# ChristophReich1996/Semantic_Pyramid_for_Image_Generation

Hardware: AMD Instinct MI355X
Metric: images/sec full G+D train step, 256x256, bs/GPU=20 (higher is better)
Workload: dtype bf16

## Files before the change

semantic_pyramid_for_image_generation_amd/csrc/conv_igemm.hip:

```cpp
#include "conv_common.h"

namespace {

template <typename T, int WCO, int WPX, int FCO, int FPX>
__global__ __launch_bounds__(256) void conv_igemm_kernel(sp_conv_params p) {
    constexpr int CO_T = WCO * FCO * 16, PX_T = WPX * FPX * 16;
    constexpr int E = 16 / (int)sizeof(T);
    constexpr int KC = 8 * E;
    constexpr int W_CH = CO_T * 8, X_CH = PX_T * 8;
    constexpr int W_PER = (W_CH + 255) / 256, X_PER = (X_CH + 255) / 256;
    constexpr int STAGE = (CO_T + PX_T) * 128;
    extern __shared__ __attribute__((aligned(16))) char smem[];

    const int tid = threadIdx.x, lane = tid & 63, wave = tid >> 6;
    const int wco = wave / WPX, wpx = wave % WPX;
    const int H = p.h, W = p.w_, CIN = p.cin_p;
    const long M = (long)p.n * H * W;
    const long px0 = (long)blockIdx.x * PX_T;
    const int co0 = blockIdx.y * CO_T;
    const int taps = p.ksize * p.ksize;
    const int kchunks = (CIN + KC - 1) / KC;
    const int nk = taps * kchunks;
    const T* __restrict__ xg = reinterpret_cast<const T*>(p.x);
    const T* __restrict__ wg = reinterpret_cast<const T*>(p.w);
// ... 675 lines not shown
        const unsigned add = c0 + ls < CIN ? (unsigned)(c0 * (int)sizeof(T)) : OOB_C;
        char* dst = halo_l + (gc & 1) * HALO_BUF + wave * 6 * 1024;
#pragma unroll
        for (int i = 0; i < 6; ++i) {
            if (wave * 6 + i < HALO_INSTR)
                __builtin_amdgcn_raw_ptr_buffer_load_lds(x_rsrc, (__attribute__((address_space(3))) void*)(dst + i * 1024), 16,
                                                         (int)(h_off[i] + add), 0, 0, 0);
        }
    };
    auto issue_w = [&](int gc, int ds, int buf) {
        const int c0 = (gc % kchunks) * KC;
        const unsigned base = (unsigned)(((TPS == 9 ? 0 : ds) * CIN + c0) * (int)sizeof(T));
        char* dst = wbuf_l + buf * W_BYTES + wave * W_PER * 1024;
#pragma unroll
        for (int i = 0; i < W_PER; ++i) {
            if (wave * W_PER + i < W_INSTR) {
                const unsigned add = c0 + w_ls(i) < CIN ? base : OOB_C;
                __builtin_amdgcn_raw_ptr_buffer_load_lds(w_rsrc, (__attribute__((address_space(3))) void*)(dst + i * 1024), 16,
                                                         (int)(w_off[i] + add), 0, 0, 0);
            }
        }
    };

    const int frow = lane & 15, fslot = lane >> 4;
    const unsigned a_addr = lds_base + 2 * HALO_BUF + (wco * 64 + (frow >> 2) * 16 + (frow & 3)) * 64 +
                            ((fslot ^ (((frow >> 1) & 1) | (((frow >> 2) & 1) << 1))) << 4);
    unsigned b_addr[3];
#pragma unroll
    for (int ds = 0; ds < 3; ++ds)
        b_addr[ds] = lds_base + ((RW * wpx) * HP + frow + ds) * 64 + ((fslot ^ (((frow + ds) >> 1) & 3)) << 4);

    const bool bias_in_acc = p.bias != nullptr && !up && p.img_scale == nullptr;
    f32x4_t acc[4][NFR];
    auto init_acc = [&](int it) {
        f32x4_t b4[4];
#pragma unroll
        for (int i = 0; i < 4; ++i) b4[i] = f32x4_t{0.f, 0.f, 0.f, 0.f};
        if (bias_in_acc && it < my_items) {
            int n, ty0, tx0, co0;
            item_coords(it, n, ty0, tx0, co0);
            const int cb = co0 + wco * 64 + (lane >> 4) * 16;
#pragma unroll
            for (int i = 0; i < 4; ++i) {
                const int co = cb + i * 4;
                if (co + 3 < p.cout) {
                    const float4 t = *reinterpret_cast<const float4*>(p.bias + co);
                    b4[i] = f32x4_t{t.x, t.y, t.z, t.w};
                } else {
#pragma unroll
                    for (int r = 0; r < 4; ++r) b4[i][r] = co + r < p.cout ? p.bias[co + r] : 0.f;
                }
            }
        }
#pragma unroll
        for (int i = 0; i < 4; ++i)
#pragma unroll
            for (int j = 0; j < NFR; ++j) acc[i][j] = b4[i];
    };
    init_acc(0);

    constexpr int IH = (WCO == 2 && RW == 4) ? 2 : 1, IW = 4 / IH;
    auto stage = [&](auto ds_c, unsigned ab, unsigned bb, auto&& mid) {
        constexpr int DS = decltype(ds_c)::value;
        constexpr int TAP_STRIDE = CO_T * 64;
        constexpr int A0 = (TPS == 9 ? DS : 0) * TAP_STRIDE, ADR = (TPS == 9 ? 3 : 1) * TAP_STRIDE;
        const unsigned bo = HP == 36 ? (bb ^ 32u) : bb;
        static_for<IH>([&](auto ihc) {
            constexpr int i0 = decltype(ihc)::value * IW;
            uint4 a[3][IW], bf[NB][2];
            static_for<IW>([&](auto i) { lds_rd128<A0 + (i0 + decltype(i)::value) * 256>(a[0][decltype(i)::value], ab); });
            lds_rd128<0>(bf[0][0], bb); lds_rd128<1024>(bf[0][1], bb);
            static_for<NB>([&](auto hc) {
                constexpr int h = decltype(hc)::value;
                if constexpr (h + 1 < NB) {
                    if constexpr (h + 1 < 3)
                        static_for<IW>([&](auto i) { lds_rd128<A0 + (h + 1) * ADR + (i0 + decltype(i)::value) * 256>(a[h + 1][decltype(i)::value], ab); });
                    lds_rd128<(h + 1) * (HP * 64)>(bf[h + 1][0], ((h + 1) & 1) ? bo : bb);
                    lds_rd128<(h + 1) * (HP * 64) + 1024>(bf[h + 1][1], ((h + 1) & 1) ? bo : bb);
                    wait_lgkm<(h + 1 < 3) ? IW + 2 : 2>();
                } else {
                    wait_lgkm<0>();
                }
                static_for<3>([&](auto drc) {
                    constexpr int dr = decltype(drc)::value;
                    constexpr int rr = h - dr;
                    if constexpr (rr >= 0 && rr < RW) {
#pragma unroll
                        for (int i = 0; i < IW; ++i)
#pragma unroll
                            for (int hh = 0; hh < 2; ++hh) Mma<T>::run(a[dr][i], bf[h][hh], acc[i0 + i][rr * 2 + hh]);
                    }
                });
                if constexpr (h == 1 && decltype(ihc)::value == 0) mid();
            });
        });
    };

    if (nchunks <= 0) return;
    const bool late = stagger != 0 && wave >= 4;
    set_halo_desc(0);
    set_w_desc(0);
    issue_halo(0);
    issue_w(0, 0, 0);
    int g = 0;
    int kc = 0, item = 0;
    const bool vec_ok = ((p.ldy & 3) == 0) && ((p.cout & 3) == 0);
    for (int gc = 0; gc < nchunks; ++gc) {
        const bool more_chunks = gc + 1 < nchunks;
        const bool item_ends = kc + 1 == kchunks;
        const unsigned hb = (unsigned)((gc & 1) * HALO_BUF);
        static_for<SPC>([&](auto sc) {
            constexpr int st = decltype(sc)::value;
            wait_vmcnt<0>();
            __builtin_amdgcn_s_barrier();
            auto request = [&]() {
                if (st + 1 < SPC) {
                    issue_w(gc, st + 1, (g + 1) & 1);
                } else if (more_chunks) {
                    if (item_ends) set_w_desc(item + 1);
                    issue_w(gc + 1, 0, (g + 1) & 1);
                }
                if (st == 0 && more_chunks) {
                    if (item_ends) set_halo_desc(item + 1);
                    issue_halo(gc + 1);
                }
            };
            if (!late) request();
            const unsigned ab = a_addr + (unsigned)((g & 1) * W_BYTES);
            auto deferred = [&]() { if (late) request(); };
            auto nothing = []() {};
            if constexpr (SPC == 3) {
                stage(std::integral_constant<int, st>{}, ab, b_addr[st] + hb, deferred);
            } else {
                stage(std::integral_constant<int, 0>{}, ab, b_addr[0] + hb, deferred);
                stage(std::integral_constant<int, 1>{}, ab, b_addr[1] + hb, nothing);
                stage(std::integral_constant<int, 2>{}, ab, b_addr[2] + hb, nothing);
            }
            ++g;
        });
        if (item_ends) {
            int n, ty0, tx0, co0;
            item_coords(item, n, ty0, tx0, co0);
            const long pix0 = ((long)n * H + ty0 + RW * wpx) * W + tx0 + (lane & 15);
            const int co_b = co0 + wco * 64 + (lane >> 4) * 16;
            const bool wide = vec_ok && (p.ldy & 7) == 0 && co_b + 16 <= p.cout;
            if (up) {
#pragma unroll
                for (int i = 0; i < 4; ++i)
#pragma unroll
                    for (int j = 0; j < NFR; ++j) acc[i][j] *= 0.25f;
            }
            static_for<NFR>([&](auto jc) {
                constexpr int j = decltype(jc)::value;
                const long pix = pix0 + (long)(j >> 1) * W + (j & 1) * 16;
                if (p.pool2) {
                    if constexpr ((j & 3) == 0) {
                        const long prow = ((long)n * (H >> 1) + ((ty0 + RW * wpx + (j >> 1)) >> 1)) * (W >> 1);
                        if constexpr (IDX) {
                            float a0[16], a1[16], b0[16], b1[16];
#pragma unroll
                            for (int i = 0; i < 4; ++i)
#pragma unroll
                                for (int r = 0; r < 4; ++r) {
                                    a0[i * 4 + r] = acc[i][j][r]; a1[i * 4 + r] = acc[i][j + 2][r];
                                    b0[i * 4 + r] = acc[i][j + 1][r]; b1[i * 4 + r] = acc[i][j + 3][r];
                                }
                            conv_epilogue_pool2_idx<T>(p, a0, a1, b0, b1, lane, prow, tx0 >> 1, co_b, !bias_in_acc);
                        } else {
                            float a[16], b[16];
#pragma unroll
                            for (int i = 0; i < 4; ++i)
#pragma unroll
                                for (int r = 0; r < 4; ++r) {
                                    a[i * 4 + r] = pool2_combine(acc[i][j][r], acc[i][j + 2][r], p.pool2 == 2);
                                    b[i * 4 + r] = pool2_combine(acc[i][j + 1][r], acc[i][j + 3][r], p.pool2 == 2);
                                }
                            conv_epilogue_pool2<T>(p, a, b, lane, prow, tx0 >> 1, co_b, !bias_in_acc);
                        }
                    }
                } else if (wide) {
                    float v[16];
#pragma unroll
                    for (int i = 0; i < 4; ++i)
#pragma unroll
                        for (int r = 0; r < 4; ++r) v[i * 4 + r] = acc[i][j][r];
                    conv_epilogue16<T>(p, v, pix, co_b, !bias_in_acc);
                } else {
#pragma unroll
                    for (int i = 0; i < 4; ++i) {
                        const int co = co_b + i * 4;
                        if (co < p.cout) {
                            float v[4] = {acc[i][j][0], acc[i][j][1], acc[i][j][2], acc[i][j][3]};
                            conv_epilogue4<T>(p, v, pix, co, vec_ok, !bias_in_acc);
                        }
                    }
                }
            });
            kc = 0;
            ++item;
            init_acc(item);
        } else {
            ++kc;
        }
    }
}

template <typename T, int WCO, int TH = 16, bool IDX = false>
int launch_tall(const sp_conv_params& p, hipStream_t s) {
    constexpr int HP = WCO == 1 ? 36 : 40;
    constexpr int LDS = 2 * ((((TH + 2) * HP * 64 + 1023) / 1024) * 1024) + 2 * (WCO == 1 ? 9 : 3) * 64 * WCO * 64;
    constexpr auto kern = conv3x3_tall_kernel<T, WCO, TH, IDX>;
    if (const int rc = sp_lds_limit<kern>(LDS)) return rc;
    const int cotiles = (p.cout + 64 * WCO - 1) / (64 * WCO);
    const int total = p.n * (p.h / TH) * (p.w_ / TL_TW) * cotiles;
    int grid = total < NUM_CU ? total : NUM_CU;
    if (grid >= 8) grid -= grid % 8;
    sp_note_route(conv_route_name(WCO == 1 ? CK_TALL_1_16 : TH == 16 ? CK_TALL_2_16 : CK_TALL_2_8, 0, sizeof(T) == 4));
    hipLaunchKernelGGL(kern, dim3((unsigned)grid), dim3(512), LDS, s, p, cotiles, total, sp_tune(SP_TUNE_CONV_STAGGER, (WCO == 2 && TH == 16) ? 1 : 0));
    SP_LAUNCH_CHECK();
    return SP_OK;
}

inline int igemm_nk(int cin_p, int ksize, int dtype) {
    const int e = dtype == SP_F32 ? 4 : 8;
    return ksize * ksize * ((cin_p + 8 * e - 1) / (8 * e));
}
inline int igemm_small_tile(long M, int cout, int cin_p, int ksize, int dtype) {
    const int forced = sp_tune(SP_TUNE_IGEMM_TILE, -1);
    if (forced >= 0) return forced;
    const long tiles64 = ((M + 63) / 64) * ((cout + 63) / 64);
    return (tiles64 > 256 && tiles64 <= 512 && igemm_nk(cin_p, ksize, dtype) >= 48 && cout % 128 == 0) ? 2 : 0;
}
struct IgemmTile { int co_t, px_t; };
constexpr int tile_key(int co_t, int px_t) { return co_t * 1024 + px_t; }
inline IgemmTile igemm_tile(bool dma, long M, int cout, int cin_p, int ksize, int dtype) {
    if (cout <= 64) return {cout <= 16 ? 16 : cout <= 32 ? 32 : 64, 256};
    if (M > 8192) return {128, 128};
    switch (dma ? igemm_small_tile(M, cout, cin_p, ksize, dtype) : 0) {
        case 1: return {128, 128};
        case 2: return {128, 64};
        case 3: return {64, 128};
        default: return {64, 64};
    }
}

inline int split_k_plan(int tiles, int nk) {
    const int target = sp_tune(SP_TUNE_SPLITK_TARGET, 384);
    int min_steps = sp_tune(SP_TUNE_SPLITK_MINSTEPS, 6);
    if (min_steps < 1) min_steps = 1;
    if (tiles > 256 || nk < 16) return 1;
    int ksplit = (target + tiles - 1) / tiles;
    if (ksplit > nk / min_steps) ksplit = nk / min_steps;
    if (ksplit > 16) ksplit = 16;
    return ksplit < 1 ? 1 : ksplit;
}
inline int igemm_ksplit_wanted(IgemmTile t, long M, int cout, int cin_p, int ksize, int dtype) {
    return split_k_plan((int)((M + t.px_t - 1) / t.px_t) * ((cout + t.co_t - 1) / t.co_t), igemm_nk(cin_p, ksize, dtype));
}
inline int igemm_ksplit(const sp_conv_params& p, IgemmTile t) {
    const long M = (long)p.n * p.h * p.w_;
    int ksplit = p.workspace == nullptr ? 1 : igemm_ksplit_wanted(t, M, p.cout, p.cin_p, p.ksize, p.dtype);
    while (ksplit > 1 && p.workspace_bytes < (int64_t)ksplit * M * p.cout * 4) --ksplit;
    if (ksplit > 1) {
        const int nk = igemm_nk(p.cin_p, p.ksize, p.dtype), per = (nk + ksplit - 1) / ksplit;
        ksplit = (nk + per - 1) / per;
    }
    return ksplit;
}

template <typename T, int WCO, int WPX, int FCO, int FPX>
int launch_dma(const sp_conv_params& p, int ksplit, hipStream_t s) {
    constexpr int CO_T = WCO * FCO * 16, PX_T = WPX * FPX * 16;
    constexpr int LDS = 3 * (CO_T + PX_T) * 128;
    constexpr auto kern = conv_igemm_dma_kernel<T, WCO, WPX, FCO, FPX>;
    if (const int rc = sp_lds_limit<kern>(LDS)) return rc;
    const long M = (long)p.n * p.h * p.w_;
    dim3 grid((unsigned)((M + PX_T - 1) / PX_T), (unsigned)((p.cout + CO_T - 1) / CO_T), (unsigned)ksplit);
    sp_note_route(conv_route_name(CK_IGEMM_DMA, ksplit > 1 ? CV_SPLITK : 0, false));
    hipLaunchKernelGGL(kern, grid, dim3(256), LDS, s, p, ksplit);
    SP_LAUNCH_CHECK();
    if (ksplit > 1) {
        long blocks = (M * ((p.cout + 3) / 4) + 255) / 256;
        if (blocks > 1024) blocks = 1024;
        hipLaunchKernelGGL(conv_finalize_kernel<T>, dim3((unsigned)blocks), dim3(256), 0, s, p, ksplit);
        SP_LAUNCH_CHECK();
    }
    return SP_OK;
}

template <typename T, int WCO, int WPX, int FCO, int FPX>
int launch_cfg(const sp_conv_params& p, hipStream_t s) {
    constexpr int CO_T = WCO * FCO * 16, PX_T = WPX * FPX * 16;
    constexpr int LDS = 2 * (CO_T + PX_T) * 128;
    constexpr auto kern = conv_igemm_kernel<T, WCO, WPX, FCO, FPX>;
    if (const int rc = sp_lds_limit<kern>(LDS)) return rc;
    const long M = (long)p.n * p.h * p.w_;
    dim3 grid((unsigned)((M + PX_T - 1) / PX_T), (unsigned)((p.cout + CO_T - 1) / CO_T));
    sp_note_route(conv_route_name(CK_IGEMM, 0, false));
    hipLaunchKernelGGL(kern, grid, dim3(256), LDS, s, p);
    SP_LAUNCH_CHECK();
    return SP_OK;
}

__global__ __launch_bounds__(256) void conv1x1_direct_kernel(sp_conv_params p, int row_bytes) {
    extern __shared__ __attribute__((aligned(16))) char wsm[];
    const int tid = threadIdx.x, lane = tid & 63, wave = tid >> 6;
    const int CIN = p.cin_p;
    const long M = (long)p.n * p.h * p.w_;
    const int co0 = blockIdx.y * 64;
    const bf16* __restrict__ xg = reinterpret_cast<const bf16*>(p.x);
    const bf16* __restrict__ wg = reinterpret_cast<const bf16*>(p.w);
    const int ksteps = (CIN + 31) / 32;
    const int cpr = ksteps * 4;
    for (int e = tid; e < 64 * cpr; e += 256) {
        const int row = e / cpr, c = e - row * cpr;
        uint4 v = make_uint4(0, 0, 0, 0);
        if (co0 + row < p.cout && c * 8 < CIN) v = *reinterpret_cast<const uint4*>(wg + (long)(co0 + row) * CIN + c * 8);
        *reinterpret_cast<uint4*>(wsm + row * row_bytes + ((c ^ (((row >> 4) & 1) << 2)) << 4)) = v;
    }
    __syncthreads();
    const int i16 = lane & 15, g = lane >> 4;
    const int arow = (i16 >> 2) * 16 + (i16 & 3);
    const int aswz = ((arow >> 4) & 1) << 2;
    const bool vec_ok = ((p.ldy & 3) == 0) && ((p.cout & 3) == 0);
    const int co_b = co0 + g * 16;
    const bool wide = vec_ok && (p.ldy & 7) == 0 && co_b + 16 <= p.cout;
    const long ngroups = (M + 31) / 32;
    for (long grp = (long)blockIdx.x * 4 + wave; grp < ngroups; grp += (long)gridDim.x * 4) {
        const long px0 = grp * 32 + i16, px1 = px0 + 16;
        const bf16* x0 = xg + (px0 < M ? px0 : M - 1) * CIN + g * 8;
        const bf16* x1 = xg + (px1 < M ? px1 : M - 1) * CIN + g * 8;
        f32x4_t acc[4][2];
#pragma unroll
        for (int i = 0; i < 4; ++i) { acc[i][0] = f32x4_t{0.f, 0.f, 0.f, 0.f}; acc[i][1] = f32x4_t{0.f, 0.f, 0.f, 0.f}; }
        for (int m = 0; m < ksteps; ++m) {
            uint4 b0 = make_uint4(0, 0, 0, 0), b1 = make_uint4(0, 0, 0, 0);
            if (m * 32 + g * 8 < CIN) {
                b0 = *reinterpret_cast<const uint4*>(x0 + m * 32);
                b1 = *reinterpret_cast<const uint4*>(x1 + m * 32);
            }
            const int slot = (m * 4 + g) ^ aswz;
#pragma unroll
            for (int i = 0; i < 4; ++i) {
                const uint4 a = *reinterpret_cast<const uint4*>(wsm + (arow + i * 4) * row_bytes + (slot << 4));
                acc[i][0] = __builtin_amdgcn_mfma_f32_16x16x32_bf16(__builtin_bit_cast(bf16x8_t, a), __builtin_bit_cast(bf16x8_t, b0), acc[i][0], 0, 0, 0);
                acc[i][1] = __builtin_amdgcn_mfma_f32_16x16x32_bf16(__builtin_bit_cast(bf16x8_t, a), __builtin_bit_cast(bf16x8_t, b1), acc[i][1], 0, 0, 0);
            }
        }
        static_for<2>([&](auto jc) {
            constexpr int j = decltype(jc)::value;
            const long pix = j == 0 ? px0 : px1;
            if (pix < M) {
                if (wide) {
                    float v[16];
#pragma unroll
                    for (int i = 0; i < 4; ++i)
#pragma unroll
                        for (int r = 0; r < 4; ++r) v[i * 4 + r] = acc[i][j][r];
                    conv_epilogue16<bf16>(p, v, pix, co_b);
                } else {
                    static_for<4>([&](auto ic) {
                        constexpr int i = decltype(ic)::value;
                        const int co = co_b + i * 4;
                        if (co < p.cout) {
                            float v[4] = {acc[i][j][0], acc[i][j][1], acc[i][j][2], acc[i][j][3]};
                            conv_epilogue4<bf16>(p, v, pix, co, vec_ok);
                        }
                    });
                }
            }
        });
    }
}

int launch_1x1_direct(const sp_conv_params& p, hipStream_t s) {
    const int ksteps = (p.cin_p + 31) / 32;
    const int row_bytes = ((ksteps * 64 + 127) / 128) * 128 + 16;
    const int lds = 64 * row_bytes;
    if (const int rc = sp_lds_limit<conv1x1_direct_kernel>(lds)) return rc;
    const long M = (long)p.n * p.h * p.w_;
    const int cotiles = (p.cout + 63) / 64;
    long gx = (M + 127) / 128;
    const long cap = 1024 / cotiles > 0 ? 1024 / cotiles : 1;
    if (gx > cap) gx = cap;
    sp_note_route(conv_route_name(CK_1X1_DIRECT, 0, false));
    hipLaunchKernelGGL(conv1x1_direct_kernel, dim3((unsigned)gx, (unsigned)cotiles), dim3(256), lds, s, p, row_bytes);
    SP_LAUNCH_CHECK();
    return SP_OK;
}


template <int KMAX>
__global__ __launch_bounds__(256) void conv1x1_splitk_kernel(sp_conv_params p) {
    __shared__ float4 red[4 * 4 * 2 * 64];
    const int tid = threadIdx.x, lane = tid & 63, wave = tid >> 6;
    const int CIN = p.cin_p;
    const long M = (long)p.n * p.h * p.w_;
    const int co0 = blockIdx.y * 64;
    const bf16* __restrict__ xg = reinterpret_cast<const bf16*>(p.x);
    const bf16* __restrict__ wg = reinterpret_cast<const bf16*>(p.w);
    const int ksteps = (CIN + 31) / 32;
    const int per = (ksteps + 3) / 4;
    const int m0 = wave * per;
    const int cnt = ksteps - m0 < per ? ksteps - m0 : per;
    const int i16 = lane & 15, g = lane >> 4;
    const int arow = (i16 >> 2) * 16 + (i16 & 3);
    const long px0 = (long)blockIdx.x * 32 + i16, px1 = px0 + 16;
    const bf16* x0 = xg + (px0 < M ? px0 : M - 1) * CIN + g * 8;
    const bf16* x1 = xg + (px1 < M ? px1 : M - 1) * CIN + g * 8;
    const bf16* wr[4];
#pragma unroll
    for (int i = 0; i < 4; ++i) {
        const int row = co0 + arow + i * 4;
        wr[i] = wg + (long)(row < p.cout ? row : p.cout - 1) * CIN + g * 8;
    }
    f32x4_t acc[4][2];
#pragma unroll
    for (int i = 0; i < 4; ++i) { acc[i][0] = f32x4_t{0.f, 0.f, 0.f, 0.f}; acc[i][1] = f32x4_t{0.f, 0.f, 0.f, 0.f}; }
    for (int c0 = 0; c0 < cnt; c0 += KMAX) {
        uint4 a[KMAX][4], b[KMAX][2];
        static_for<KMAX>([&](auto uc) {
            constexpr int u = decltype(uc)::value;
            const int m = m0 + c0 + u;
#pragma unroll
            for (int i = 0; i < 4; ++i) a[u][i] = make_uint4(0, 0, 0, 0);
            b[u][0] = make_uint4(0, 0, 0, 0);
            b[u][1] = make_uint4(0, 0, 0, 0);
            if (c0 + u < cnt && m * 32 + g * 8 < CIN) {
#pragma unroll
                for (int i = 0; i < 4; ++i) a[u][i] = *reinterpret_cast<const uint4*>(wr[i] + m * 32);
                b[u][0] = *reinterpret_cast<const uint4*>(x0 + m * 32);
                b[u][1] = *reinterpret_cast<const uint4*>(x1 + m * 32);
            }
        });
        static_for<KMAX>([&](auto uc) {
            constexpr int u = decltype(uc)::value;
            if (c0 + u < cnt) {
#pragma unroll
                for (int i = 0; i < 4; ++i) {
                    acc[i][0] = __builtin_amdgcn_mfma_f32_16x16x32_bf16(__builtin_bit_cast(bf16x8_t, a[u][i]), __builtin_bit_cast(bf16x8_t, b[u][0]), acc[i][0], 0, 0, 0);
                    acc[i][1] = __builtin_amdgcn_mfma_f32_16x16x32_bf16(__builtin_bit_cast(bf16x8_t, a[u][i]), __builtin_bit_cast(bf16x8_t, b[u][1]), acc[i][1], 0, 0, 0);
                }
            }
        });
    }
#pragma unroll
    for (int i = 0; i < 4; ++i)
#pragma unroll
        for (int j = 0; j < 2; ++j)
            red[((wave * 4 + i) * 2 + j) * 64 + lane] = make_float4(acc[i][j][0], acc[i][j][1], acc[i][j][2], acc[i][j][3]);
    __syncthreads();
    const bool vec_ok = ((p.ldy & 3) == 0) && ((p.cout & 3) == 0);
    const int co = co0 + g * 16 + wave * 4;
    if (co >= p.cout) return;
#pragma unroll
    for (int j = 0; j < 2; ++j) {
        const long pix = j == 0 ? px0 : px1;
        float v[4] = {0.f, 0.f, 0.f, 0.f};
#pragma unroll
        for (int src = 0; src < 4; ++src) {
            const float4 t = red[((src * 4 + wave) * 2 + j) * 64 + lane];
            v[0] += t.x; v[1] += t.y; v[2] += t.z; v[3] += t.w;
        }
        if (pix < M) conv_epilogue4<bf16>(p, v, pix, co, vec_ok);
    }
}

int launch_1x1_splitk(const sp_conv_params& p, hipStream_t s) {
    const int ksteps = (p.cin_p + 31) / 32;
    const long M = (long)p.n * p.h * p.w_;
    dim3 grid((unsigned)((M + 31) / 32), (unsigned)((p.cout + 63) / 64));
    sp_note_route(conv_route_name(CK_1X1_SPLITK, 0, false));
    if (ksteps <= 8) hipLaunchKernelGGL(conv1x1_splitk_kernel<2>, grid, dim3(256), 0, s, p);
    else if (ksteps <= 16) hipLaunchKernelGGL(conv1x1_splitk_kernel<4>, grid, dim3(256), 0, s, p);
    else hipLaunchKernelGGL(conv1x1_splitk_kernel<6>, grid, dim3(256), 0, s, p);
    SP_LAUNCH_CHECK();
    return SP_OK;
}

constexpr int C8_TH = 16, C8_TW = 32, C8_HW = C8_TW + 2, C8_HH = C8_TH + 2;

__global__ __launch_bounds__(256) void conv3x3_cin8_kernel(sp_conv_params p) {
    __shared__ __attribute__((aligned(16))) uint4 halo[C8_HH * C8_HW];
    const int tid = threadIdx.x, lane = tid & 63, wave = tid >> 6;
    const int H = p.h, W = p.w_;
    const int tiles_x = W / C8_TW, tiles_y = H / C8_TH;
    int t = blockIdx.x;
    const int tx0 = (t % tiles_x) * C8_TW; t /= tiles_x;
    const int ty0 = (t % tiles_y) * C8_TH;
    const int n = t / tiles_y;
    const uint4* __restrict__ xg = reinterpret_cast<const uint4*>(p.x);
    const uint4* __restrict__ wg = reinterpret_cast<const uint4*>(p.w);
    uint4 hv[3];
#pragma unroll
    for (int q = 0; q < 3; ++q) {
        const int e = tid + q * 256;
        const int r = e / C8_HW, c = e - r * C8_HW;
        const int y = ty0 - 1 + r, x = tx0 - 1 + c;
        hv[q] = make_uint4(0, 0, 0, 0);
        if (e < C8_HH * C8_HW && (unsigned)y < (unsigned)H && (unsigned)x < (unsigned)W) hv[q] = xg[((long)n * H + y) * W + x];
    }
    const int i16 = lane & 15, g = lane >> 4;
    uint4 a[4][3];
#pragma unroll
    for (int i = 0; i < 4; ++i) {
        const int co = (i16 >> 2) * 16 + i * 4 + (i16 & 3);
#pragma unroll
        for (int m = 0; m < 3; ++m) {
            const int tap = m * 4 + g;
            a[i][m] = make_uint4(0, 0, 0, 0);
            if (tap < 9 && co < p.cout) a[i][m] = wg[co * 9 + tap];
        }
    }
#pragma unroll
    for (int q = 0; q < 3; ++q) {
        const int e = tid + q * 256;
        if (e < C8_HH * C8_HW) halo[e] = hv[q];
    }
    __syncthreads();
    int toff[3];
#pragma unroll
    for (int m = 0; m < 3; ++m) {
        const int tap = m * 4 + g < 9 ? m * 4 + g : 8;
        toff[m] = (tap / 3) * C8_HW + tap % 3;
    }
    const int co_b = g * 16;
    const bool co_ok = co_b + 16 <= p.cout;
    float bias[16];
#pragma unroll
    for (int r = 0; r < 16; ++r) bias[r] = 0.f;
    if (p.bias && co_ok) Wide16<float>::ld(p.bias + co_b, bias);
#pragma unroll 2
    for (int rr = 0; rr < C8_TH / 4; ++rr) {
        const int row = wave * (C8_TH / 4) + rr;
        f32x4_t acc[4][2];
#pragma unroll
        for (int i = 0; i < 4; ++i) { acc[i][0] = f32x4_t{0.f, 0.f, 0.f, 0.f}; acc[i][1] = f32x4_t{0.f, 0.f, 0.f, 0.f}; }
#pragma unroll
        for (int m = 0; m < 3; ++m) {
            const uint4 b0 = halo[row * C8_HW + i16 + toff[m]];
            const uint4 b1 = halo[row * C8_HW + 16 + i16 + toff[m]];
#pragma unroll
            for (int i = 0; i < 4; ++i) {
                acc[i][0] = __builtin_amdgcn_mfma_f32_16x16x32_bf16(__builtin_bit_cast(bf16x8_t, a[i][m]), __builtin_bit_cast(bf16x8_t, b0), acc[i][0], 0, 0, 0);
                acc[i][1] = __builtin_amdgcn_mfma_f32_16x16x32_bf16(__builtin_bit_cast(bf16x8_t, a[i][m]), __builtin_bit_cast(bf16x8_t, b1), acc[i][1], 0, 0, 0);
            }
        }
        if (!co_ok) continue;
        const long pix0 = ((long)n * H + ty0 + row) * W + tx0 + i16;
        const float sc = conv_img_scale(p, pix0);
#pragma unroll
        for (int j = 0; j < 2; ++j) {
            float v[16];
#pragma unroll
            for (int i = 0; i < 4; ++i)
#pragma unroll
                for (int r = 0; r < 4; ++r) v[i * 4 + r] = acc[i][j][r] * sc + bias[i * 4 + r];
            conv_epilogue16<bf16>(p, v, pix0 + j * 16, co_b, false);
        }
    }
}

int launch_cin8(const sp_conv_params& p, hipStream_t s) {
    const long blocks = (long)p.n * (p.h / C8_TH) * (p.w_ / C8_TW);
    sp_note_route(conv_route_name(CK_CIN8, 0, false));
    hipLaunchKernelGGL(conv3x3_cin8_kernel, dim3((unsigned)blocks), dim3(256), 0, s, p);
    SP_LAUNCH_CHECK();
    return SP_OK;
}

constexpr int TN_TH = 8, TN_TW = 32, TN_HW = TN_TW + 2, TN_HH = TN_TH + 2;

template <int KC>
__global__ __launch_bounds__(256) void conv3x3_thinco_kernel(sp_conv_params p) {
    extern __shared__ __attribute__((aligned(16))) char tn_smem[];
    constexpr int CIN = KC * 32, PITCH = CIN * 2 + 16, CPP = KC * 4;
    constexpr int NCH = TN_HH * TN_HW * CPP, PER = (NCH + 255) / 256;
    const int tid = threadIdx.x, lane = tid & 63, wave = tid >> 6;
    const int H = p.h, W = p.w_;
    const int tiles_x = W / TN_TW, tiles_y = H / TN_TH;
    int t = blockIdx.x;
    const int tx0 = (t % tiles_x) * TN_TW; t /= tiles_x;
    const int ty0 = (t % tiles_y) * TN_TH;
    const int n = t / tiles_y;
    const uint4* __restrict__ xg = reinterpret_cast<const uint4*>(p.x);
    const uint4* __restrict__ wg = reinterpret_cast<const uint4*>(p.w);
    uint4 hv[PER];
#pragma unroll
    for (int q = 0; q < PER; ++q) {
        const int e = tid + q * 256;
        const int px = e / CPP, c = e - px * CPP;
        const int r = px / TN_HW, cc = px - r * TN_HW;
        const int y = ty0 - 1 + r, x = tx0 - 1 + cc;
        hv[q] = make_uint4(0, 0, 0, 0);
        if (e < NCH && (unsigned)y < (unsigned)H && (unsigned)x < (unsigned)W) hv[q] = xg[(((long)n * H + y) * W + x) * CPP + c];
    }
    const int i16 = lane & 15, g = lane >> 4;
    uint4 a[9][KC];
#pragma unroll
    for (int tap = 0; tap < 9; ++tap)
#pragma unroll
        for (int kc = 0; kc < KC; ++kc) {
            a[tap][kc] = make_uint4(0, 0, 0, 0);
            if (i16 < p.cout) a[tap][kc] = wg[(i16 * 9 + tap) * CPP + kc * 4 + g];
        }
#pragma unroll
    for (int q = 0; q < PER; ++q) {
        const int e = tid + q * 256;
        const int px = e / CPP, c = e - px * CPP;
        if (e < NCH) *reinterpret_cast<uint4*>(tn_smem + px * PITCH + c * 16) = hv[q];
    }
    __syncthreads();
    const bool vec_ok = ((p.ldy & 3) == 0) && ((p.cout & 3) == 0);
#pragma unroll
    for (int rr = 0; rr < TN_TH / 4; ++rr) {
        const int row = wave * (TN_TH / 4) + rr;
        f32x4_t acc[2] = {f32x4_t{0.f, 0.f, 0.f, 0.f}, f32x4_t{0.f, 0.f, 0.f, 0.f}};
#pragma unroll
        for (int tap = 0; tap < 9; ++tap) {
            const char* base = tn_smem + ((row + tap / 3) * TN_HW + i16 + tap % 3) * PITCH + g * 16;
#pragma unroll
            for (int kc = 0; kc < KC; ++kc) {
                const uint4 b0 = *reinterpret_cast<const uint4*>(base + kc * 64);
                const uint4 b1 = *reinterpret_cast<const uint4*>(base + 16 * PITCH + kc * 64);
                acc[0] = __builtin_amdgcn_mfma_f32_16x16x32_bf16(__builtin_bit_cast(bf16x8_t, a[tap][kc]), __builtin_bit_cast(bf16x8_t, b0), acc[0], 0, 0, 0);
                acc[1] = __builtin_amdgcn_mfma_f32_16x16x32_bf16(__builtin_bit_cast(bf16x8_t, a[tap][kc]), __builtin_bit_cast(bf16x8_t, b1), acc[1], 0, 0, 0);
            }
        }
        if (g != 0) continue;
        const long pix0 = ((long)n * H + ty0 + row) * W + tx0 + i16;
#pragma unroll
        for (int j = 0; j < 2; ++j) {
            float v[4] = {acc[j][0], acc[j][1], acc[j][2], acc[j][3]};
            conv_epilogue4<bf16>(p, v, pix0 + j * 16, 0, vec_ok);
        }
    }
}

template <int KC>
int launch_thinco(const sp_conv_params& p, hipStream_t s) {
    constexpr int LDS = TN_HH * TN_HW * (KC * 64 + 16);
    if (const int rc = sp_lds_limit<conv3x3_thinco_kernel<KC>>(LDS)) return rc;
    const long blocks = (long)p.n * (p.h / TN_TH) * (p.w_ / TN_TW);
    sp_note_route(conv_route_name(CK_THINCO, 0, false));
    hipLaunchKernelGGL(conv3x3_thinco_kernel<KC>, dim3((unsigned)blocks), dim3(256), LDS, s, p);
    SP_LAUNCH_CHECK();
    return SP_OK;
}

inline bool conv_halo_path(long M, int h, int w, int cin_p, int cout, int ksize) {
    const bool thin_big = cout <= 16 && cin_p >= 32 && M >= (1L << 18);
    return ksize == 3 && (cout > 32 || thin_big) && h % HALO_TH == 0 && w % HALO_TW == 0;
}
inline bool conv_w16_path(int w, int cout, int ksize, bool h16) {
    const int ppm = sp_tune(SP_TUNE_CONV_PP, 1);
    return h16 && ksize == 3 && w == 16 && cout > 64 && (ppm == 1 || ppm == 3);
}
inline bool conv_dma_path(long M, int cout, int ksize) {
    const int dma_mode = sp_tune(SP_TUNE_IGEMM_DMA, 1);
    return cout > 16 && (dma_mode == 2 || (dma_mode == 1 && ksize == 3 && M <= 8192));
}

ConvRoute conv_plan(const sp_conv_params& p) {
    const auto route = [](int kernel, int form = 0) { return ConvRoute{kernel, form, 0, 0, 1, nullptr}; };
    const auto unsupported = [](const char* msg) { return ConvRoute{CK_UNSUPPORTED, 0, 0, 0, 1, msg}; };
    int form;
    if (p.dtype == SP_F8) {
        if ((form = sp_conv_pp_form(p, CK_PP_8ROW)) >= 0) return route(CK_PP_8ROW, form);
        return unsupported("sp_conv2d_igemm: SP_F8 covers 3x3 layers with cout > 64, h %% 8 == 0, w %% 32 == 0 only");
    }
    const bool h16 = p.dtype != SP_F32;
    const int esz = h16 ? 2 : 4, idx = p.pool_idx != nullptr ? CV_IDX : 0;
    const int pp_mode = h16 ? sp_tune(SP_TUNE_CONV_PP, 1) : 0, tall_mode = sp_tune(SP_TUNE_CONV_TALL, 1);
    if (p.tail_w != nullptr) {
        if (!p.in_up2 && p.img_scale == nullptr && pp_mode && tall_mode == 1 && (form = sp_conv_pp_form(p, CK_PP_16ROW)) >= 0) return route(CK_PP_16ROW, form);
        return unsupported("sp_conv2d_igemm: the fused 1x1 tail needs 16-bit storage, a 3x3 layer with cout == 64, h %% 16 == 0, w %% 32 == 0, ldy %% 8 == 0, no pooling");
    }
    const long M = (long)p.n * p.h * p.w_;
    if (h16 && p.ksize == 3 && p.cout <= 4 && (p.cin_p == 32 || p.cin_p == 64) && !p.pool2 && !p.in_up2 && p.h % TN_TH == 0 &&
        p.w_ % TN_TW == 0 && sp_tune(SP_TUNE_CONV_THINCO, 1) && tall_mode <= 1)
        return route(CK_THINCO);
    if (h16 && p.ksize == 3 && p.cin_p == 8 && p.cout % 16 == 0 && p.cout <= 64 && (p.ldy & 7) == 0 && !p.pool2 && !p.in_up2 &&
        p.h % C8_TH == 0 && p.w_ % C8_TW == 0 && sp_tune(SP_TUNE_CONV_CIN8, 1) && tall_mode <= 1)
        return route(CK_CIN8);
    if (h16 && p.ksize == 1) {
        const int ks = (p.cin_p + 31) / 32;
        const bool few_blocks = ((M + 31) / 32) * ((p.cout + 63) / 64) <= sp_tune(SP_TUNE_CONV1X1_SPLITK, 320);
        if (few_blocks && (p.cin_p > 1024 || (ks >= 4 && ks <= 24))) return route(CK_1X1_SPLITK);
        if (p.cin_p <= 1024 && sp_tune(SP_TUNE_CONV1X1_DIRECT, 1)) return route(CK_1X1_DIRECT);
    }
    const bool fits30 = conv_operands_below_1g(p, esz);
// ... 158 lines not shown
```

Before: 1366.

## Pipeline 1x1 direct conv with register-prefetched activations and templated K depth

Rewrites the 1x1 direct convolution kernel so the K depth is a template parameter. Activation loads for all K steps are issued into registers up front, and the next pixel group is prefetched while the current epilogue runs; a ring mode streams batches for deep channel counts. Weight loading into LDS is overlapped with the first activation loads, and the grid is sized from the CU count and LDS occupancy instead of a fixed cap. The costs are heavier register pressure, more template instantiations, and reliance on inline asm and sched barriers.

Measured after the change: 1372 (median of 6 runs). About the same (+0.4%).

```diff
diff --git a/semantic_pyramid_for_image_generation_amd/csrc/conv_igemm.hip b/semantic_pyramid_for_image_generation_amd/csrc/conv_igemm.hip
--- a/semantic_pyramid_for_image_generation_amd/csrc/conv_igemm.hip
+++ b/semantic_pyramid_for_image_generation_amd/csrc/conv_igemm.hip
@@ -1001,54 +1001,141 @@
     return SP_OK;
 }
 
-__global__ __launch_bounds__(256) void conv1x1_direct_kernel(sp_conv_params p, int row_bytes) {
+inline long direct1x1_ranges(long M, int cotiles, int lds_bytes) {
+    int per_cu = (160 * 1024) / lds_bytes;
+    per_cu = per_cu > 4 ? 4 : per_cu < 1 ? 1 : per_cu;
+    const long groups = (M + 31) / 32;
+    long ranges = (long)NUM_CU * per_cu / cotiles;
+    if (ranges > 8) ranges &= ~7L;
+    if (ranges > (groups + 3) / 4) ranges = (groups + 3) / 4;
+    return ranges < 1 ? 1 : ranges;
+}
+
+template <int KB, bool RING>
+__global__ __launch_bounds__(256, RING && KB == 8 ? 2 : 4) void conv1x1_direct_kernel(sp_conv_params p, int row_bytes, int nranges, int nbatch) {
     extern __shared__ __attribute__((aligned(16))) char wsm[];
-    const int tid = threadIdx.x, lane = tid & 63, wave = tid >> 6;
+    const int tid = threadIdx.x, lane = tid & 63;
+    const int wave = __builtin_amdgcn_readfirstlane(tid >> 6);
     const int CIN = p.cin_p;
     const long M = (long)p.n * p.h * p.w_;
-    const int co0 = blockIdx.y * 64;
-    const bf16* __restrict__ xg = reinterpret_cast<const bf16*>(p.x);
-    const bf16* __restrict__ wg = reinterpret_cast<const bf16*>(p.w);
-    const int ksteps = (CIN + 31) / 32;
-    const int cpr = ksteps * 4;
-    for (int e = tid; e < 64 * cpr; e += 256) {
-        const int row = e / cpr, c = e - row * cpr;
-        uint4 v = make_uint4(0, 0, 0, 0);
-        if (co0 + row < p.cout && c * 8 < CIN) v = *reinterpret_cast<const uint4*>(wg + (long)(co0 + row) * CIN + c * 8);
-        *reinterpret_cast<uint4*>(wsm + row * row_bytes + ((c ^ (((row >> 4) & 1) << 2)) << 4)) = v;
-    }
+    const int cotiles = (p.cout + 63) >> 6;
+    const int bq = (int)blockIdx.x >> 3;
+    const int range = (bq / cotiles) * 8 + ((int)blockIdx.x & 7);
+    if (range >= nranges) return;
+    const int co0 = (bq % cotiles) * 64;
+    const int ksteps = RING ? nbatch * KB : KB;
+    int i16 = lane & 15, g = lane >> 4;
+    const int ngroups = (int)((M + 31) / 32);
+    const int gstride = nranges * 4;
+    const char* xb;
+    unsigned r0, r1;
+    auto rows_of = [&](int gr) {
+        const long p0 = (long)(gr < ngroups ? gr : ngroups - 1) * 32;
+        const int last = (int)(M - 1 - p0 < 31 ? M - 1 - p0 : 31);
+        xb = reinterpret_cast<const char*>(p.x) + p0 * CIN * 2;
+        r0 = (unsigned)((i16 < last ? i16 : last) * CIN * 2);
+        r1 = (unsigned)((i16 + 16 < last ? i16 + 16 : last) * CIN * 2);
+    };
+    uint4 b[KB][2];
+    auto issue = [&](auto jc, int base, bool may_be_last) {
+        constexpr int j = decltype(jc)::value;
+        unsigned ch = (unsigned)(base + j * 64 + g * 16);
+        if (j == KB - 1 && may_be_last) ch = ch < (unsigned)CIN * 2 ? ch : 0u;
+        b[j][0] = *reinterpret_cast<const uint4*>(xb + (r0 + ch));
+        b[j][1] = *reinterpret_cast<const uint4*>(xb + (r1 + ch));
+    };
+    constexpr int NF = RING ? 4 : (KB + 1) / 2;
+    const int kpieces = (ksteps + 1) / 2;
+    const int frow = tid >> 3, fswz = ((frow >> 4) & 1) << 2;
+    const char* wb = reinterpret_cast<const char*>(p.w) + (long)co0 * CIN * 2;
+    const int wlast = p.cout - 1 - co0;
+    uint4 wv[NF][2];
+    auto fill_issue = [&](int k0) {
+        static_for<NF>([&](auto kc) {
+            constexpr int k = decltype(kc)::value;
+            const int c8 = ((tid & 7) + 8 * (k0 + k)) * 8;
+#pragma unroll
+            for (int hf = 0; hf < 2; ++hf) {
+                const int row = frow + 32 * hf;
+                wv[k][hf] = *reinterpret_cast<const uint4*>(wb + (unsigned)(((row < wlast ? row : wlast) * CIN + (c8 < CIN ? c8 : 0)) * 2));
+            }
+        });
+    };
+    auto fill_write = [&](int k0) {
+        static_for<NF>([&](auto kc) {
+            constexpr int k = decltype(kc)::value;
+            if (!RING || k0 + k < kpieces) {
+                const int c = (tid & 7) + 8 * (k0 + k);
+#pragma unroll
+                for (int hf = 0; hf < 2; ++hf) {
+                    const int row = frow + 32 * hf;
+                    const bool live = row <= wlast && c * 8 < CIN;
+                    uint4 v = wv[k][hf];
+                    v.x = live ? v.x : 0u; v.y = live ? v.y : 0u; v.z = live ? v.z : 0u; v.w = live ? v.w : 0u;
+                    *reinterpret_cast<uint4*>(wsm + row * row_bytes + ((c ^ fswz) << 4)) = v;
+                }
+            }
+        });
+    };
+    int grp = range * 4 + wave;
+    rows_of(grp);
+    fill_issue(0);
+    static_for<KB>([&](auto jc) { issue(jc, 0, !RING); });
+    fill_write(0);
+    if (RING)
+        for (int k0 = NF; k0 < kpieces; k0 += NF) { fill_issue(k0); fill_write(k0); }
     __syncthreads();
-    const int i16 = lane & 15, g = lane >> 4;
-    const int arow = (i16 >> 2) * 16 + (i16 & 3);
-    const int aswz = ((arow >> 4) & 1) << 2;
-    const bool vec_ok = ((p.ldy & 3) == 0) && ((p.cout & 3) == 0);
-    const int co_b = co0 + g * 16;
-    const bool wide = vec_ok && (p.ldy & 7) == 0 && co_b + 16 <= p.cout;
-    const long ngroups = (M + 31) / 32;
-    for (long grp = (long)blockIdx.x * 4 + wave; grp < ngroups; grp += (long)gridDim.x * 4) {
-        const long px0 = grp * 32 + i16, px1 = px0 + 16;
-        const bf16* x0 = xg + (px0 < M ? px0 : M - 1) * CIN + g * 8;
-        const bf16* x1 = xg + (px1 < M ? px1 : M - 1) * CIN + g * 8;
+    auto group = [&](auto more_c) {
+        constexpr bool MORE = decltype(more_c)::value;
+        unsigned zero;
+        asm volatile("v_mov_b32 %0, 0" : "=v"(zero));
+        const int ln = (int)__builtin_amdgcn_mbcnt_hi(~0u, __builtin_amdgcn_mbcnt_lo(~0u, zero));
+        i16 = ln & 15; g = ln >> 4;
+        const int arow = (i16 >> 2) * 16 + (i16 & 3);
+        const int aswz = ((arow >> 4) & 1) << 2;
+        const int co_b = co0 + g * 16;
+        const bool vec_ok = ((p.ldy & 3) == 0) && ((p.cout & 3) == 0);
+        const bool wide = vec_ok && (p.ldy & 7) == 0 && co_b + 16 <= p.cout;
+        const int abase = arow * row_bytes;
         f32x4_t acc[4][2];
 #pragma unroll
         for (int i = 0; i < 4; ++i) { acc[i][0] = f32x4_t{0.f, 0.f, 0.f, 0.f}; acc[i][1] = f32x4_t{0.f, 0.f, 0.f, 0.f}; }
-        for (int m = 0; m < ksteps; ++m) {
-            uint4 b0 = make_uint4(0, 0, 0, 0), b1 = make_uint4(0, 0, 0, 0);
-            if (m * 32 + g * 8 < CIN) {
-                b0 = *reinterpret_cast<const uint4*>(x0 + m * 32);
-                b1 = *reinterpret_cast<const uint4*>(x1 + m * 32);
-            }
+        auto kstep = [&](int m, const uint4& b0, const uint4& b1) {
             const int slot = (m * 4 + g) ^ aswz;
 #pragma unroll
             for (int i = 0; i < 4; ++i) {
-                const uint4 a = *reinterpret_cast<const uint4*>(wsm + (arow + i * 4) * row_bytes + (slot << 4));
+                const uint4 a = *reinterpret_cast<const uint4*>(wsm + abase + i * 4 * row_bytes + (slot << 4));
                 acc[i][0] = __builtin_amdgcn_mfma_f32_16x16x32_bf16(__builtin_bit_cast(bf16x8_t, a), __builtin_bit_cast(bf16x8_t, b0), acc[i][0], 0, 0, 0);
                 acc[i][1] = __builtin_amdgcn_mfma_f32_16x16x32_bf16(__builtin_bit_cast(bf16x8_t, a), __builtin_bit_cast(bf16x8_t, b1), acc[i][1], 0, 0, 0);
             }
+        };
+        if (RING)
+            for (int bt = 0; bt + 1 < nbatch; ++bt) {
+                static_for<KB>([&](auto jc) {
+                    constexpr int j = decltype(jc)::value;
+                    kstep(bt * KB + j, b[j][0], b[j][1]);
+                    issue(jc, (bt + 1) * KB * 64, true);
+                    __builtin_amdgcn_sched_barrier(0);
+                });
+            }
+        static_for<KB>([&](auto jc) {
+            constexpr int j = decltype(jc)::value;
+            const int m = ksteps - KB + j;
+            uint4 b0 = b[j][0], b1 = b[j][1];
+            if (j == KB - 1) {
+                const bool live = m * 32 + g * 8 < CIN;
+                b0.x = live ? b0.x : 0u; b0.y = live ? b0.y : 0u; b0.z = live ? b0.z : 0u; b0.w = live ? b0.w : 0u;
+                b1.x = live ? b1.x : 0u; b1.y = live ? b1.y : 0u; b1.z = live ? b1.z : 0u; b1.w = live ? b1.w : 0u;
+            }
+            kstep(m, b0, b1);
+        });
+        if (MORE) {
+            rows_of(grp + gstride);
+            static_for<KB>([&](auto jc) { issue(jc, 0, !RING); });
         }
         static_for<2>([&](auto jc) {
             constexpr int j = decltype(jc)::value;
-            const long pix = j == 0 ? px0 : px1;
+            const long pix = (long)grp * 32 + j * 16 + i16;
             if (pix < M) {
                 if (wide) {
                     float v[16];
@@ -1069,23 +1156,42 @@
                 }
             }
         });
-    }
+    };
+    if (grp >= ngroups) return;
+    for (; grp + gstride < ngroups; grp += gstride) group(std::true_type{});
+    group(std::false_type{});
+}
+
+template <int KB, bool RING>
+int launch_1x1_direct_kb(const sp_conv_params& p, int ksteps, hipStream_t s) {
+    const int row_bytes = ((ksteps * 64 + 127) / 128) * 128 + 16;
+    const int lds = 64 * row_bytes;
+    if (const int rc = sp_lds_limit<conv1x1_direct_kernel<KB, RING>>(lds)) return rc;
+    const int cotiles = (p.cout + 63) / 64;
+    const long ranges = direct1x1_ranges((long)p.n * p.h * p.w_, cotiles, lds);
+    const long blocks = (ranges + 7) / 8 * 8 * cotiles;
+    sp_note_route(conv_route_name(CK_1X1_DIRECT, 0, false));
+    hipLaunchKernelGGL((conv1x1_direct_kernel<KB, RING>), dim3((unsigned)blocks), dim3(256), lds, s, p, row_bytes, (int)ranges, ksteps / KB);
+    SP_LAUNCH_CHECK();
+    return SP_OK;
 }
 
 int launch_1x1_direct(const sp_conv_params& p, hipStream_t s) {
     const int ksteps = (p.cin_p + 31) / 32;
-    const int row_bytes = ((ksteps * 64 + 127) / 128) * 128 + 16;
-    const int lds = 64 * row_bytes;
-    if (const int rc = sp_lds_limit<conv1x1_direct_kernel>(lds)) return rc;
-    const long M = (long)p.n * p.h * p.w_;
-    const int cotiles = (p.cout + 63) / 64;
-    long gx = (M + 127) / 128;
-    const long cap = 1024 / cotiles > 0 ? 1024 / cotiles : 1;
-    if (gx > cap) gx = cap;
-    sp_note_route(conv_route_name(CK_1X1_DIRECT, 0, false));
-    hipLaunchKernelGGL(conv1x1_direct_kernel, dim3((unsigned)gx, (unsigned)cotiles), dim3(256), lds, s, p, row_bytes);
-    SP_LAUNCH_CHECK();
-    return SP_OK;
+    switch (ksteps) {
+        case 1: return launch_1x1_direct_kb<1, false>(p, ksteps, s);
+        case 2: return launch_1x1_direct_kb<2, false>(p, ksteps, s);
+        case 3: return launch_1x1_direct_kb<3, false>(p, ksteps, s);
+        case 4: return launch_1x1_direct_kb<4, false>(p, ksteps, s);
+        case 5: return launch_1x1_direct_kb<5, false>(p, ksteps, s);
+        case 6: return launch_1x1_direct_kb<6, false>(p, ksteps, s);
+        case 7: return launch_1x1_direct_kb<7, false>(p, ksteps, s);
+        case 8: return launch_1x1_direct_kb<8, false>(p, ksteps, s);
+    }
+    if (ksteps % 8 == 0) return launch_1x1_direct_kb<8, true>(p, ksteps, s);
+    if (ksteps % 4 == 0) return launch_1x1_direct_kb<4, true>(p, ksteps, s);
+    if (ksteps % 2 == 0) return launch_1x1_direct_kb<2, true>(p, ksteps, s);
+    return launch_1x1_direct_kb<1, true>(p, ksteps, s);
 }
 
 
```
